# turtle-robotics/sea-current

Hardware: AMD Instinct MI355X
Metric: plans/sec (batched start-goal, 1024^2 grid) (higher is better)
Workload: dtype int32; 1 GPU; 1024x1024 random-obstacle grids (salt20, one grid and one query block per step), EDT + A*, 1024 batched queries per GPU and step, 10 steps = 10240 queries per library call; queries_per_launch=10240, map=salt20, queries_per_gpu=1024, queries_total=1024, lmax=4096, parallelism=query-sharded x1, contexts_in_flight=2, steps_per_call=10, hw_queues=4

## Files before the change

### include/sea_current_hip.h

```cpp
#ifndef SEA_CURRENT_HIP_H
#define SEA_CURRENT_HIP_H
#include <stdint.h>
#ifdef __cplusplus
extern "C" {
#endif

#define SC_ABI_VERSION 1

typedef struct sc_ctx sc_ctx;

typedef enum {
    SC_OK = 0,
    SC_ERR_INVALID = 1,
    SC_ERR_HIP = 2,
    SC_ERR_NOMEM = 3,
    SC_ERR_NO_DEVICE = 4
} sc_status;

typedef enum {
    SC_Q_OK = 0,
    SC_Q_NO_PATH = 1,
    SC_Q_BAD_ENDPOINT = 2,
    SC_Q_TRUNCATED = 3,
    SC_Q_RING_OVERFLOW = 4,
// ... 31 lines not shown
int sc_ctx_set_stream(sc_ctx* ctx, void* hip_stream);
int sc_ctx_use_own_stream(sc_ctx* ctx);
int sc_ctx_synchronize(sc_ctx* ctx);
int sc_ctx_set_timing(sc_ctx* ctx, int enable);
int sc_ctx_reset_timing(sc_ctx* ctx);
int sc_ctx_get_timing(sc_ctx* ctx, int kernel_id, double* total_ms, int64_t* launches);
int sc_ctx_scratch_bytes(sc_ctx* ctx, int64_t* bytes);

int sc_edt_u8_i32(sc_ctx* ctx, const uint8_t* occ, int W, int H, int batch, int32_t* d2);
int sc_edt_u8_i32_host(sc_ctx* ctx, const uint8_t* occ, int W, int H, int batch, int32_t* d2);

int sc_edt_nearest_i32(sc_ctx* ctx, const uint8_t* occ, const int32_t* d2, int W, int H, int batch, int32_t* nearest);

int sc_occ_from_rects(sc_ctx* ctx, const uint8_t* base, const int32_t* rects, int R, int W, int H, int free_border, uint8_t* occ);

int sc_occ_from_polygons(sc_ctx* ctx, const uint8_t* base, int G, int W, int H, float x_min, float y_min, float res_x, float res_y,
                         const float* lines, int n_lines, const int32_t* obs_off, int n_obs, const float* obs_box,
                         const uint8_t* obs_closed, const int32_t* grid_off, uint8_t* occ);
int sc_occ_from_polygons_host(sc_ctx* ctx, const uint8_t* base, int G, int W, int H, float x_min, float y_min, float res_x,
                              float res_y, const float* lines, int n_lines, const int32_t* obs_off, int n_obs, const float* obs_box,
                              const uint8_t* obs_closed, const int32_t* grid_off, uint8_t* occ);

int sc_moves_i32_u8(sc_ctx* ctx, const int32_t* d2, int W, int H, int32_t r2_clear, uint8_t* moves);

int sc_astar_batch(sc_ctx* ctx, const int32_t* d2, int W, int H, int32_t r2_clear,
                   const int32_t* start, const int32_t* goal, int Q, int Lmax,
                   int32_t* path, int32_t* len, int32_t* cost, int32_t* status);
int sc_astar_batch_host(sc_ctx* ctx, const int32_t* d2, int W, int H, int32_t r2_clear,
                        const int32_t* start, const int32_t* goal, int Q, int Lmax,
                        int32_t* path, int32_t* len, int32_t* cost, int32_t* status);
int sc_astar_batch_multi(sc_ctx* ctx, const int32_t* d2, int G, const int32_t* qgrid, int W, int H, int32_t r2_clear,
                         const int32_t* start, const int32_t* goal, int Q, int Lmax,
                         int32_t* path, int32_t* len, int32_t* cost, int32_t* status);
int sc_astar_last_expansions(sc_ctx* ctx, int64_t* expansions);
int sc_astar_debug_stats(sc_ctx* ctx, int32_t* stats4, int Q);
int sc_astar_debug_peek(sc_ctx* ctx, int32_t* out16);
int sc_astar_gfield(sc_ctx* ctx, const int32_t* d2, int W, int H, int32_t r2_clear,
                    int32_t start, int32_t goal, uint32_t* gfield, int32_t* cost, int32_t* status);

#define SC_FIELD_INF INT32_MAX
int sc_cost_field_batch(sc_ctx* ctx, const int32_t* d2, int G, const int32_t* fgrid, int W, int H, int32_t r2_clear,
                        const int32_t* root, int F, int rounds, int32_t* g, int32_t* fstatus);
int sc_cost_field_batch_host(sc_ctx* ctx, const int32_t* d2, int G, const int32_t* fgrid, int W, int H, int32_t r2_clear,
                             const int32_t* root, int F, int rounds, int32_t* g, int32_t* fstatus);
int sc_field_paths_batch(sc_ctx* ctx, const int32_t* d2, int G, const int32_t* fgrid, int W, int H, int32_t r2_clear,
                         const int32_t* g, const int32_t* root, int F, const int32_t* qfield, const int32_t* target, int Q,
// ... 406 lines not shown
```

### sea-current_amd/csrc/astar.hip

```cpp
#include "sc_internal.h"
#include <stdlib.h>

#define NBUCKET 32
#define ASTAR_CQ_THROUGHPUT 1024
#define ASTAR_RU_THROUGHPUT 4
#define ASTAR_CQ_LATENCY 2048
#define ASTAR_RU_LATENCY 8
#define E_RUN (1u << 18)
#define E_START (4u << 13 | 3u << 16)
#define RUNK 8

struct astar_args {
    const uint8_t* moves;
    const int32_t* d2;
    int W, H;
    int32_t rmin;
    const int32_t* start;
    const int32_t* goal;
    const int32_t* qgrid;
    const int32_t* order;
    const int32_t* nq_dev;
    int nq;
    int Lmax;
    int32_t* path;
    int32_t* len;
    int32_t* cost;
    int32_t* status;
    void* g;
    uint32_t* closed;
    uint32_t* buckets;
    int cap;
    int32_t* expanded;
    int32_t* counter;
    int32_t* ovf_list;
    int32_t* ovf_count;
    int32_t* ovf_sticky;
    int nstat;
    int lazy;
    int tw, bw;
    size_t gcells, bwords;
};

__device__ __forceinline__ int octile(int x, int y, int gx, int gy) {
    int dx = abs(x - gx), dy = abs(y - gy);
    return 10 * max(dx, dy) + 4 * min(dx, dy);
}

__device__ __forceinline__ uint32_t gix(int x, int y, int tw) {
    return ((((uint32_t)(y >> 2) * (uint32_t)tw + (uint32_t)(x >> 2)) << 4) | ((uint32_t)(y & 3) << 2)) | (uint32_t)(x & 3);
}
__device__ __forceinline__ uint32_t gix8(int x, int y, int tw8) {
    return ((((uint32_t)(y >> 3) * (uint32_t)tw8 + (uint32_t)(x >> 3)) << 6) | ((uint32_t)(y & 7) << 3)) | (uint32_t)(x & 7);
}
template <typename GT> __device__ __forceinline__ uint32_t gidx(int x, int y, int tw);
template <> __device__ __forceinline__ uint32_t gidx<uint32_t>(int x, int y, int tw) { return gix(x, y, tw); }
template <> __device__ __forceinline__ uint32_t gidx<uint8_t>(int x, int y, int tw) { return gix8(x, y, tw); }
__device__ __forceinline__ uint32_t cix(int x, int y, int bw) {
    return (((uint32_t)(y >> 4) * (uint32_t)bw + (uint32_t)(x >> 5)) << 4) | (uint32_t)(y & 15);
}

template <typename T>
__device__ __forceinline__ T g_load(const T* p) {
    return __hip_atomic_load(p, __ATOMIC_RELAXED, __HIP_MEMORY_SCOPE_AGENT);
// ... 60 lines not shown
                 "global_load_ubyte %[m], %[ma], off\n\t"
                 "s_mov_b64 %[sv], exec\n\t"
                 "v_cmp_ne_u32_e32 vcc, 0, %[b]\n\t"
                 "s_and_b64 exec, %[sv], vcc\n\t"
                 "global_atomic_or %[o], %[a], %[b], off sc0\n\t"
                 "s_mov_b64 exec, %[sv]"
                 : [sv] "=&s"(sv), [o] "+v"(old), [m] "=&v"(pmv), [r0] "=&v"(rm[0]), [r1] "=&v"(rm[1]), [r2] "=&v"(rm[2]), [r3] "=&v"(rm[3]),
                   [r4] "=&v"(rm[4]), [r5] "=&v"(rm[5]), [r6] "=&v"(rm[6])
                 : [a] "v"(bit_addr), [b] "v"(bits), [ma] "v"(mv_addr), [p0] "v"(ra[0]), [p1] "v"(ra[1]), [p2] "v"(ra[2]), [p3] "v"(ra[3]),
                   [p4] "v"(ra[4]), [p5] "v"(ra[5]), [p6] "v"(ra[6])
                 : "vcc", "scc", "memory");
}
__device__ __forceinline__ void pop_run_wait_loads(uint32_t (&rm)[RUNK - 1], uint32_t& pmv, uint32_t& old) {
    asm volatile("s_waitcnt vmcnt(1)" : "+v"(pmv), "+v"(old), "+v"(rm[0]), "+v"(rm[1]), "+v"(rm[2]), "+v"(rm[3]), "+v"(rm[4]), "+v"(rm[5]), "+v"(rm[6]) : : "memory");
}
__device__ __forceinline__ void pop_pair_wait_load(uint32_t& pmv, uint32_t& old) { asm volatile("s_waitcnt vmcnt(1)" : "+v"(pmv), "+v"(old) : : "memory"); }

__device__ __forceinline__ void pop_loads_issue(const uint8_t* mv_addr, const uint32_t* w_addr, uint32_t& byte, uint32_t& word) {
    asm volatile("global_load_ubyte %0, %2, off\n\t"
                 "global_load_dword %1, %3, off sc1"
                 : "=&v"(byte), "=&v"(word) : "v"(mv_addr), "v"(w_addr) : "memory");
}
__device__ __forceinline__ void pop_loads_wait(uint32_t& byte, uint32_t& word) { asm volatile("s_waitcnt vmcnt(0)" : "+v"(byte), "+v"(word) : : "memory"); }
__device__ __forceinline__ void masked_or_noret(uint32_t* addr, uint32_t bits) {
    unsigned long long sv;
    asm volatile("s_mov_b64 %[sv], exec\n\t"
                 "v_cmp_ne_u32_e32 vcc, 0, %[b]\n\t"
                 "s_and_b64 exec, %[sv], vcc\n\t"
                 "global_atomic_or %[a], %[b], off\n\t"
                 "s_mov_b64 exec, %[sv]"
                 : [sv] "=&s"(sv) : [a] "v"(addr), [b] "v"(bits) : "vcc", "scc", "memory");
}

__device__ __forceinline__ uint32_t bcast_group8(uint32_t v) {
    const uint32_t q = (uint32_t)__builtin_amdgcn_update_dpp(0, (int)v, 0x00 , 0xF, 0xF, false);
    const uint32_t r = (uint32_t)__builtin_amdgcn_update_dpp(0, (int)q, 0x114 , 0xF, 0xF, false);
    return q | r;
}

#define HQ 256
#define ASTAR_SPIN_LIMIT (1 << 20)
template <typename GT, bool DUAL, int CQ, int REFILL_UNROLL>
__device__ __forceinline__ void astar_query(const astar_args& a, const int q, const int slot) {
    constexpr int REFILL = CQ / 2;
    __shared__ uint32_t qe[CQ + 64];
    __shared__ int s_head[NBUCKET];
    __shared__ int s_tail[NBUCKET];
    __shared__ uint32_t nd_xy[64];
    __shared__ uint32_t nd_mv[64];
    __shared__ uint16_t succ[512];
    __shared__ uint8_t prune_tbl[64];
    __shared__ uint32_t dup_tbl[DUAL ? 1024 + 64 : 1];
    __shared__ uint2 hq_rec[DUAL ? HQ + 64 : 1];
    __shared__ int hq_tail, hq_head, hq_clean, hq_stop, hq_ovf, hq_fcur, hq_found, hq_flush;
    constexpr int SCOPE = DUAL ? __HIP_MEMORY_SCOPE_WORKGROUP : __HIP_MEMORY_SCOPE_WAVEFRONT;
    const int lane = threadIdx.x & 63;
    const int wv = DUAL ? __builtin_amdgcn_readfirstlane((int)(threadIdx.x >> 6)) : 0;
    const int W = a.W, H = a.H;
    const size_t cells = (size_t)W * H;
    const int s = a.start[q], t = a.goal[q];
    int32_t* path = a.path + (size_t)q * a.Lmax;

    int out_st = SC_Q_OK, out_len = 0, out_cost = -1, nexp = 0, npop = 0, kcyc = 0, nstep = 0;
    const size_t grid_off = a.qgrid ? (size_t)a.qgrid[q] * cells : 0;
    const uint8_t* const mvs = a.moves + grid_off;
    const bool bad = s < 0 || t < 0 || (size_t)s >= cells || (size_t)t >= cells || a.d2[grid_off + s] < a.rmin || a.d2[grid_off + t] < a.rmin;
    if (bad) out_st = SC_Q_BAD_ENDPOINT;
    else if (s == t) {
        if (lane == 0 && wv == 0) path[0] = s;
        out_len = 1; out_cost = 0; nexp = 1;
    } else {
    const int tw = a.tw, bw = a.bw;
    GT* g = static_cast<GT*>(a.g) + (size_t)slot * a.gcells;
    uint32_t* cl = a.closed + (size_t)slot * a.bwords;
    uint32_t* bk = a.buckets + (size_t)slot * NBUCKET * a.cap;
    const int cap = a.cap, capm = a.cap - 1;
    const int sx = s % W, sy = s / W, gx = t % W, gy = t / W;
    const int ddx[8] = {1, -1, 0, 0, 1, -1, 1, -1};
    const int ddy[8] = {0, 0, 1, -1, 1, 1, -1, -1};

    {
        uint4* p = reinterpret_cast<uint4*>(cl);
        const size_t n4 = a.bwords >> 2;
        for (size_t i = DUAL ? threadIdx.x : lane; i < n4; i += DUAL ? 128 : 64) p[i] = make_uint4(0, 0, 0, 0);
    }
    __builtin_amdgcn_wave_barrier();
    if (wv == 0 && lane < NBUCKET) { s_head[lane] = 0; s_tail[lane] = 0; }
    if (wv == 0) prune_tbl[lane] = (uint8_t)entry_prune((uint32_t)lane << 13);
// ... 217 lines not shown
                lt += n;
                if (lane == 0) __hip_atomic_store(&s_head[b], hd + n, __ATOMIC_RELAXED, SCOPE);
                wave_lds_sync();
            }
            const int n = min(64, lt - lh);
            npop += n; ++nstep;
            if (DUAL && n <= 16) {
                const int kl = n <= 4 ? 3 : n <= 8 ? 2 : n <= 16 ? 1 : 0, KL = 1 << kl, GL = 2 * KL;
                const int sub = lane >> (kl + 1), j = (lane >> kl) & 1, k = lane & (KL - 1);
                const bool valid = sub < n;
                const uint32_t e_raw = qe[(lh + sub) & (CQ - 1)];
                const uint32_t e = valid ? e_raw : 0u;
                lh += n;
                const int x = e & 0x1FFF, y = e >> 19;
                const uint32_t bit = 1u << (x & 31);
                const int dxg = gx - x, dyg = gy - y, adx = abs(dxg), ady = abs(dyg);
                const int dD = 4 + ((dxg < 0 ? 1 : 0) | (dyg < 0 ? 2 : 0));
                const int dS = adx > ady ? (dxg < 0 ? 1 : 0) : (dyg < 0 ? 3 : 2);
                const uint32_t bD = adx >= 1 && ady >= 1 ? 1u << dD : 0u, bS = adx != ady ? 1u << dS : 0u;
                const int d = j ? dS : dD;
                const bool has = valid && (j ? bS : bD) != 0u;
                const int lgeom = j ? abs(adx - ady) : min(adx, ady);
                const int ddx_ = (int)((0x2252u >> (2 * d)) & 3u) - 1, ddy_ = (int)((0x0A25u >> (2 * d)) & 3u) - 1;
                const uint8_t* const addr = mvs + (y * W + x) + (has ? min(k, lgeom - 1) : 0) * (ddy_ * W + ddx_);
                const bool head = valid && j == 0 && k == 0;
                uint32_t old, byte;
                uint32_t* const wa = &cl[cix(x, y, bw)];
                pop_loads_issue(addr, wa, byte, old);
                const uint32_t prune = prune_tbl[(e >> 13) & 63u];
                const int dup = dup_settle(head, x, y, e);
                pop_loads_wait(byte, old);
                const bool link = has && k < lgeom && ((byte >> d) & 1u) && (k > 0 || !((prune >> d) & 1u));
                const unsigned long long lm = __ballot(link);
                const uint32_t grp = (uint32_t)(lm >> (lane & ~(KL - 1))) & ((1u << KL) - 1u);
                const int run = __ffs((int)~grp) - 1;
                const uint32_t ne = entry_pack(x + (k + 1) * ddx_, y + (k + 1) * ddy_, d, byte) | (k + 1 < run ? E_RUN : 0u);
                const bool won1 = head && dup == 0 && !(old & bit);
                masked_or_noret(wa, won1 ? bit : 0u);
                const unsigned long long wm1 = __ballot(won1);
                const bool act = ((wm1 >> (lane & ~(GL - 1))) & 1ull) && k < run;
                {
                    const unsigned long long ma = __ballot(act);
                    if (ma) {
                        const int c = __popcll(ma);
                        if (__builtin_expect(lt - lh + c <= CQ, 1)) {
                            qe[act ? ((lt + (int)__builtin_amdgcn_mbcnt_hi((uint32_t)(ma >> 32), __builtin_amdgcn_mbcnt_lo((uint32_t)ma, 0u))) & (CQ - 1)) : CQ + lane] = ne;
                            lt += c;
                        } else push_entry(act, ne, 0);
                    }
                }
                hand_over(won1, x, y, (byte & ~prune) & ~(bD | bS), byte);
                nexp += __popcll(wm1);
            } else if (!DUAL && n <= 8) {
                const int sub = lane >> 3, d = lane & 7;
                const bool valid = sub < n;
                const uint32_t e = valid ? qe[(lh + sub) & (CQ - 1)] : 0u;
                lh += n;
                const int x = e & 0x1FFF, y = e >> 19;
                const uint32_t bit = 1u << (x & 31);
                uint32_t old = 0, pmv;
                const int hc = octile(x, y, gx, gy);
// ... 17 lines not shown
                    if (run == k && k < lmax && ((rm[k - 1] >> d) & 1u)) run = k + 1;
                const uint32_t ne = entry_pack(nx, ny, d, pmv) | (run > 1 ? E_RUN : 0u);
                atomic_wait(old);
                old = bcast_group8(old);
                const bool won = valid && !(old & bit);
                push_entry(won && cand, ne, df);
#pragma unroll
                for (int k = 2; k <= RUNK; ++k) {
                    if (__ballot(won && run >= k) == 0) break;
                    push_entry(won && run >= k, entry_pack(x + k * mdx, y + k * mdy, d, rm[k - 2]) | (run > k ? E_RUN : 0u), 0);
                }
                nexp += __popcll(__ballot(won && d == 0));
                if (__ballot(won && x == gx && y == gy)) found = true;
                if (won && d == 0) g[gidx<GT>(x, y, tw)] = (GT)(fcur - hc);
            } else if (DUAL) {
                const bool valid = lane < n;
                const uint32_t e_raw = qe[(lh + lane) & (CQ - 1)];
                const uint32_t e = valid ? e_raw : 0u;
                lh += n;
                const int x = e & 0x1FFF, y = e >> 19;
                const uint32_t bit = 1u << (x & 31);
                uint32_t old, pmv;
                uint32_t* const wa = &cl[cix(x, y, bw)];
                pop_loads_issue(mvs + (y * W + x), wa, pmv, old);
                const int dup = dup_settle(valid, x, y, e);
                const uint32_t prune = prune_tbl[(e >> 13) & 63u];
                const int dxg = gx - x, dyg = gy - y, adx = abs(dxg), ady = abs(dyg);
                const int dD = 4 + ((dxg < 0 ? 1 : 0) | (dyg < 0 ? 2 : 0));
                const int dS = adx > ady ? (dxg < 0 ? 1 : 0) : (dyg < 0 ? 3 : 2);
                const uint32_t bD = adx >= 1 && ady >= 1 ? 1u << dD : 0u, bS = adx != ady ? 1u << dS : 0u;
                const int nxD = x + (dxg < 0 ? -1 : 1), nyD = y + (dyg < 0 ? -1 : 1);
                const int nxS = x + (adx > ady ? (dxg < 0 ? -1 : 1) : 0), nyS = y + (adx > ady ? 0 : (dyg < 0 ? -1 : 1));
                pop_loads_wait(pmv, old);
                const uint32_t cand = valid ? (pmv & ~prune) : 0u;
                const uint32_t neD = (uint32_t)nyD << 19 | (uint32_t)dD << 13 | (uint32_t)nxD;
                const uint32_t neS = entry_pack(nxS, nyS, dS, pmv);
                const bool won = valid && dup == 0 && !(old & bit);
                masked_or_noret(wa, won ? bit : 0u);
                {
                    const bool pD = won && (cand & bD), pS = won && (cand & bS);
                    const unsigned long long mD = __ballot(pD), mS = __ballot(pS);
                    const int cD = __popcll(mD), c2 = cD + __popcll(mS);
                    if (c2) {
                        if (__builtin_expect(lt - lh + c2 <= CQ, 1)) {
                            qe[pD ? ((lt + (int)__builtin_amdgcn_mbcnt_hi((uint32_t)(mD >> 32), __builtin_amdgcn_mbcnt_lo((uint32_t)mD, 0u))) & (CQ - 1)) : CQ + lane] = neD;
                            qe[pS ? ((lt + cD + (int)__builtin_amdgcn_mbcnt_hi((uint32_t)(mS >> 32), __builtin_amdgcn_mbcnt_lo((uint32_t)mS, 0u))) & (CQ - 1)) : CQ + lane] = neS;
                            lt += c2;
                        } else {
                            push_entry(pD, neD, 0);
                            push_entry(pS, neS, 0);
                        }
                    }
                }
                nexp += __popcll(hand_over(won, x, y, cand & ~(bD | bS), pmv));
            } else {
                const bool valid = lane < n;
                const uint32_t e = valid ? qe[(lh + lane) & (CQ - 1)] : 0u;
                lh += n;
                const int x = e & 0x1FFF, y = e >> 19;
                const uint32_t bit = 1u << (x & 31);
                uint32_t old = 0, pmv;
// ... 147 lines not shown
            }
            out_len = L; out_cost = fcur;
        }
    }
    kcyc = (int)((__builtin_amdgcn_s_memtime() - t_begin) >> 10);
    }
    if (lane == 0 && wv == 0) {
        a.status[q] = out_st; a.len[q] = out_len; a.cost[q] = out_cost;
        a.expanded[q] = nexp; a.expanded[a.nstat + q] = npop; a.expanded[2 * a.nstat + q] = kcyc; a.expanded[3 * a.nstat + q] = nstep;
    }
}

template <typename GT>
__global__ void __launch_bounds__(64) astar_kernel(astar_args a) {
    const int nq = a.nq_dev ? *a.nq_dev : a.nq;
    for (;;) {
        const int qi = __builtin_amdgcn_readfirstlane(atomicAdd(a.counter, 1)) >> 6;
        if (qi >= nq) break;
        astar_query<GT, false, ASTAR_CQ_THROUGHPUT, ASTAR_RU_THROUGHPUT>(a, a.order ? a.order[qi] : qi, (int)blockIdx.x);
    }
}

template <typename GT, int CQ, int RU>
__global__ void __launch_bounds__(128) astar_kernel_dual(astar_args a) {
    __shared__ int s_qi;
    const int nq = a.nq_dev ? *a.nq_dev : a.nq;
    for (;;) {
        if (threadIdx.x == 0) s_qi = atomicAdd(a.counter, 64) >> 6;
        __syncthreads();
        const int qi = __builtin_amdgcn_readfirstlane(s_qi);
        __syncthreads();
        if (qi >= nq) break;
        astar_query<GT, true, CQ, RU>(a, a.order ? a.order[qi] : qi, (int)blockIdx.x);
        __syncthreads();
    }
}

__global__ void __launch_bounds__(1024) astar_prep_kernel(const int32_t* __restrict__ start, const int32_t* __restrict__ goal, int Q, int W,
                                                          int H, int32_t* __restrict__ order, int32_t* __restrict__ ctr) {
    __shared__ int hist[1024];
    __shared__ int scan[1024];
    const int tid = threadIdx.x;
    if (tid < 4) ctr[tid] = 0;
    if (!order) return;
    hist[tid] = 0;
    __syncthreads();
    const int hmax = 14 * max(W, H) + 1;
// ... 92 lines not shown
    if (slots * gcells * gsz > ctx->gslots.bytes || slots * bwords * 4 > ctx->closed.bytes || ring_slots(slots) * NBUCKET * (size_t)cap * 4 > ctx->buckets.bytes) {
        size_t free_b = 0, total_b = 0;
        if (hipMemGetInfo(&free_b, &total_b) == hipSuccess) {
            const size_t avail = (size_t)(0.9 * (double)(free_b + ctx->gslots.bytes + ctx->closed.bytes + ctx->buckets.bytes));
            while (slots > 1 && slots * (gcells * gsz + bwords * 4) + ring_slots(slots) * NBUCKET * (size_t)cap * 4 > avail) slots = (slots + 1) / 2;
        }
    }
    for (;;) {
        r = sc_scratch_reserve(ctx, &ctx->gslots, slots * gcells * gsz);
        if (r == SC_OK) r = sc_scratch_reserve(ctx, &ctx->closed, slots * bwords * 4);
        if (r == SC_OK) r = sc_scratch_reserve(ctx, &ctx->buckets, ring_slots(slots) * NBUCKET * (size_t)cap * 4);
        if (r == SC_OK) break;
        if (r != SC_ERR_NOMEM || slots <= 1) return r;
        (void)hipGetLastError();
        slots = (slots + 1) / 2;
    }
    if (!ctx->actr.p) {
        r = sc_scratch_reserve(ctx, &ctx->actr, 16 * sizeof(int32_t));
        if (r != SC_OK) return r;
        SC_HIP(ctx, hipMemsetAsync(ctx->actr.p, 0, 16 * sizeof(int32_t), ctx->stream));
    }
    int32_t* ctr = (int32_t*)ctx->actr.p;
    ctx->status_armed = true;

    const bool sorted = (size_t)Q > slots;
    int tk = sc_time_begin(ctx, SC_K_ASTAR);
    hipLaunchKernelGGL(astar_prep_kernel, dim3(1), dim3(1024), 0, ctx->stream, start, goal, Q, W, H, sorted ? order : (int32_t*)nullptr, ctr);
    astar_args a{(const uint8_t*)ctx->moves.p, d2, W, H, rmin, start, goal, qgrid, sorted ? order : nullptr, nullptr, Q, Lmax, path, len,
                 cost, status, ctx->gslots.p, (uint32_t*)ctx->closed.p, (uint32_t*)ctx->buckets.p, cap, expanded, ctr,
                 ovf_list, ctr + 1, ctx->status + SC_ST_ASTAR_OVERFLOW, Q, (dual && (size_t)Q > slots) ? 1 : 0, tw, bw, gcells, bwords};
    if (full_g) hipLaunchKernelGGL(astar_kernel<uint32_t>, dim3((unsigned)slots), dim3(64), 0, ctx->stream, a);
    else if (dual && latency && (size_t)Q <= slots)
        hipLaunchKernelGGL((astar_kernel_dual<uint8_t, ASTAR_CQ_LATENCY, ASTAR_RU_LATENCY>), dim3((unsigned)slots), dim3(128), 0, ctx->stream, a);
    else if (dual)
        hipLaunchKernelGGL((astar_kernel_dual<uint8_t, ASTAR_CQ_THROUGHPUT, ASTAR_RU_THROUGHPUT>), dim3((unsigned)slots), dim3(128), 0, ctx->stream, a);
    else hipLaunchKernelGGL(astar_kernel<uint8_t>, dim3((unsigned)slots), dim3(64), 0, ctx->stream, a);
    {
        const size_t rslots = slots >= 16 ? slots / 16 : 1;
        const int rcap = cap * 16;
        astar_args b = a;
        b.order = ovf_list; b.nq_dev = ctr + 1; b.nq = 0; b.cap = rcap; b.counter = ctr + 2;
        b.ovf_list = order; b.ovf_count = ctr + 3;
        if (full_g) hipLaunchKernelGGL(astar_kernel<uint32_t>, dim3((unsigned)rslots), dim3(64), 0, ctx->stream, b);
        else hipLaunchKernelGGL(astar_kernel<uint8_t>, dim3((unsigned)rslots), dim3(64), 0, ctx->stream, b);
    }
    sc_time_end(ctx, tk);
    SC_HIP(ctx, hipGetLastError());
    return SC_OK;
}

extern "C" int sc_astar_batch(sc_ctx* ctx, const int32_t* d2, int W, int H, int32_t r2_clear,
                              const int32_t* start, const int32_t* goal, int Q, int Lmax,
                              int32_t* path, int32_t* len, int32_t* cost, int32_t* status) {
// ... 69 lines not shown
```

### sea-current_amd/csrc/moves.hip

```cpp
#include "sc_internal.h"

__global__ void __launch_bounds__(256)
moves_kernel(const int32_t* __restrict__ d2, int W, int Hall, int H, int32_t rmin, uint8_t* __restrict__ moves) {
    const int x = blockIdx.x * 256 + threadIdx.x;
    const int yall = blockIdx.y;
    if (x >= W) return;
    const int y = yall % H;
    const int32_t* r1 = d2 + (size_t)yall * W;
    bool t[3][3];
#pragma unroll
    for (int j = -1; j <= 1; ++j)
#pragma unroll
        for (int i = -1; i <= 1; ++i) {
            int xx = x + i, yy = y + j;
            t[j + 1][i + 1] = xx >= 0 && xx < W && yy >= 0 && yy < H && r1[(ptrdiff_t)j * W + xx] >= rmin;
        }
    uint32_t m = 0;
    if (t[1][1]) {
        m |= (uint32_t)t[1][2] << 0;
        m |= (uint32_t)t[1][0] << 1;
        m |= (uint32_t)t[2][1] << 2;
        m |= (uint32_t)t[0][1] << 3;
        m |= (uint32_t)(t[2][2] && t[1][2] && t[2][1]) << 4;
        m |= (uint32_t)(t[2][0] && t[1][0] && t[2][1]) << 5;
// ... 73 lines not shown
    }
}

int sc_launch_moves(sc_ctx* ctx, const int32_t* d2, int W, int Hall, int H, int32_t r2, uint8_t* moves) {
    int32_t rmin = r2 > 1 ? r2 : 1;
    int tk = sc_time_begin(ctx, SC_K_MOVES);
    if (W % 4 == 0 && H % 4 == 0 && ((uintptr_t)d2 & 15) == 0 && ((uintptr_t)moves & 3) == 0)
        hipLaunchKernelGGL(moves4x4_kernel, dim3((W / 4 + 255) / 256, Hall / 4), dim3(256), 0, ctx->stream, d2, W, Hall, H, rmin, moves);
    else if (W % 4 == 0 && ((uintptr_t)d2 & 15) == 0 && ((uintptr_t)moves & 3) == 0)
        hipLaunchKernelGGL(moves4_kernel, dim3((W / 4 + 255) / 256, Hall), dim3(256), 0, ctx->stream, d2, W, Hall, H, rmin, moves);
    else
        hipLaunchKernelGGL(moves_kernel, dim3((W + 255) / 256, Hall), dim3(256), 0, ctx->stream, d2, W, Hall, H, rmin, moves);
    sc_time_end(ctx, tk);
    SC_HIP(ctx, hipGetLastError());
    return SC_OK;
}

extern "C" int sc_moves_i32_u8(sc_ctx* ctx, const int32_t* d2, int W, int H, int32_t r2_clear, uint8_t* moves) {
    if (!ctx || !d2 || !moves || W <= 0 || H <= 0 || W > SC_MAX_DIM || H > SC_MAX_DIM) return SC_ERR_INVALID;
    SC_HIP(ctx, hipSetDevice(ctx->device));
    return sc_launch_moves(ctx, d2, W, H, H, r2_clear, moves);
}

__host__ __device__ static inline int64_t isqrt64(int64_t v) {
    int64_t r = (int64_t)sqrt((double)v);
    while (r * r > v) --r;
    while ((r + 1) * (r + 1) <= v) ++r;
    return r;
}

__global__ void __launch_bounds__(256)
clearance_penalty_kernel(const int32_t* __restrict__ d2, size_t n, int32_t thr, int32_t r2_soft, int64_t s10, int pen_max,
                         uint8_t* __restrict__ pen) {
    const size_t i = (size_t)blockIdx.x * 256 + threadIdx.x;
    if (i >= n) return;
    const int32_t d = d2[i];
    uint8_t p = 0;
    if (d >= thr && d < r2_soft) p = (uint8_t)(((int64_t)pen_max * (s10 - isqrt64(100ll * d))) / s10);
    pen[i] = p;
}

extern "C" int sc_clearance_penalty_u8(sc_ctx* ctx, const int32_t* d2, int W, int H, int batch, int32_t r2_clear, int32_t r2_soft,
                                       int pen_max, uint8_t* pen) {
    if (!ctx || !d2 || !pen || W <= 0 || H <= 0 || W > SC_MAX_DIM || H > SC_MAX_DIM || batch <= 0 || pen_max < 0 || pen_max > 255 ||
        r2_soft < 1)
        return SC_ERR_INVALID;
// ... 25 lines not shown
```

### sea-current_amd/csrc/sc_internal.h

```cpp
#pragma once
#include <hip/hip_runtime.h>
#include <math.h>
#include <stdint.h>
#include <stdio.h>
#include <string.h>

#include <set>
#include <vector>

#include "../../include/sea_current_hip.h"

struct sc_scratch {
    void* p = nullptr;
    size_t bytes = 0;
    sc_scratch() = default;
    sc_scratch(const sc_scratch&) = delete;
    sc_scratch& operator=(const sc_scratch&) = delete;
    ~sc_scratch() { if (p) (void)hipFree(p); }
};

static inline size_t al256(size_t b) { return (b + 255) & ~(size_t)255; }

enum sc_status_word {
    SC_ST_ASTAR_OVERFLOW,
// ... 4 lines not shown
};

struct __attribute__((visibility("hidden"))) sc_ctx {
    int device = 0;
    hipStream_t own_stream = nullptr;
    hipStream_t stream = nullptr;
    hipEvent_t wait_ev = nullptr;
    int32_t *status = nullptr, *status_host = nullptr;
    bool status_armed = false;
    char err[256] = {0};
    int timing = 0;
    struct pending_ev { int kid; hipEvent_t a, b; bool shared_a = false; };
    std::vector<pending_ev> pending;
    std::vector<hipEvent_t> ev_pool;
    double t_ms[SC_K_COUNT] = {0};
    int64_t t_n[SC_K_COUNT] = {0};
    size_t scratch_total = 0;
    sc_scratch host_stage;
    sc_scratch astar_ends;
    sc_scratch colbits;
    sc_scratch updown;
    sc_scratch edt_flags;
    sc_scratch moves;
    sc_scratch gslots;
    sc_scratch closed;
    sc_scratch buckets;
    sc_scratch qstats;
    sc_scratch actr;
    sc_scratch bez_tang;
    sc_scratch bez_gl;
    sc_scratch bez_seginfo;
    sc_scratch cheb_a;
    sc_scratch fmt_nbr;
    sc_scratch gather_msg;
    sc_scratch wp_spill;
    sc_scratch sm_ctrl;
    sc_scratch sm_cum;
    sc_scratch sm_tp;
    sc_scratch sm_int;
    sc_scratch sm_smp;
    sc_scratch sm_vlim;
    sc_scratch occ_prep;
    sc_scratch fld_mask;
    sc_scratch fld_state;
    sc_scratch cmp_state;
    sc_scratch cmp_start;
// ... 70 lines not shown
    int upload();
    template <class T> T* dev(int i) const { return (T*)((char*)ctx_->host_stage.p + off_[i]); }
    int finish(int r);

  private:
    struct copy { int slot; void* host; size_t bytes; };
    int slot(size_t bytes) {
        off_.push_back(end_);
        end_ += al256(bytes ? bytes : 1);
        return (int)off_.size() - 1;
    }
    sc_ctx* ctx_;
    size_t end_ = 0;
    std::vector<size_t> off_;
    std::vector<copy> up_, down_;
};

int sc_time_begin(sc_ctx* ctx, int kid);
void sc_time_end(sc_ctx* ctx, int token);
int sc_time_chain(sc_ctx* ctx, int token, int kid);

int sc_launch_edt(sc_ctx* ctx, const uint8_t* occ, int W, int H, int batch, int32_t* d2);
int sc_launch_moves(sc_ctx* ctx, const int32_t* d2, int W, int Hall, int H, int32_t r2, uint8_t* moves);
int sc_launch_arclength(sc_ctx* ctx, const float* ctrl, int S, int nsub, float* cum, float* seg_len, const int32_t* S_dev);
int sc_launch_resample(sc_ctx* ctx, const float* ctrl, const float* cum, const float* arclength, const int32_t* seg_off, int B, int S,
                       int nsub, float* profile_pos, const int32_t* prof_off, int nudge, float* pts, float* tpar, int32_t* seg,
                       float* curvature, int32_t* status, const int32_t* S_dev);
struct sc_speed_frame {
    const int32_t* d2;
    int W, H;
    float x_min, y_min, res_x, res_y;
};
static inline bool sc_frame_ok(const sc_speed_frame& fr) {
    return fr.W >= 1 && fr.W <= SC_MAX_DIM && fr.H >= 1 && fr.H <= SC_MAX_DIM && isfinite(fr.x_min) && isfinite(fr.y_min) &&
           isfinite(fr.res_x) && fr.res_x > 0.f && isfinite(fr.res_y) && fr.res_y > 0.f;
}
int sc_launch_speed_limits(sc_ctx* ctx, const float* ctrl, const float* cum, const int32_t* seg_off, const float* arclength,
                           const int32_t* status, int P, int nsub, int N, int J, const double* limits, const double* dyn,
                           const sc_speed_frame& fr, int ns_bound, double* vlo, double* vhi, double* vhi_copy, float* min_clear,
                           int32_t* status_out);
int sc_speed_args_ok(int J, const double* dyn, const sc_speed_frame& fr);
int sc_speed_dyn_ok(const double* dyn, int P);
int sc_curve_grid_ok(const sc_speed_frame& fr, int32_t r2_clear);
int sc_launch_curve_clear(sc_ctx* ctx, const float* ctrl_in, float* ctrl_out, const int32_t* seg_off, const int32_t* status, int P,
                          const sc_speed_frame& fr, int32_t r2_clear, int max_level, uint8_t* level, int32_t* rounds, int32_t* leg_min,
                          int32_t* status_out);
// ... 31 lines not shown
```

### sea-current_amd/python/sea_current_amd/__init__.py

```python
import ctypes as C
import os
import re
import subprocess

import numpy as np

_PKG = os.path.dirname(os.path.abspath(__file__))
NATIVE_DIR = os.path.normpath(os.path.join(_PKG, "..", ".."))
REPO_ROOT = os.path.normpath(os.path.join(NATIVE_DIR, ".."))
LIB_PATH = os.environ.get("SC_LIB_PATH") or os.path.join(NATIVE_DIR, "libsea_current_hip.so")
HEADER_PATH = os.path.join(REPO_ROOT, "include", "sea_current_hip.h")

EDT_INF = 2**31 - 1
FIELD_INF = 2**31 - 1
FIELD_SEED_COST_MAX = 1 << 24
Q_OK, Q_NO_PATH, Q_BAD_ENDPOINT, Q_TRUNCATED, Q_RING_OVERFLOW, Q_BAD_PATH = 0, 1, 2, 3, 4, 5
K_EDT_COLBITS, K_EDT_BAND, K_MOVES, K_ASTAR, K_TOPPRA, K_TOPPRA_SAMPLE, K_BEZIER, K_ARCLENGTH, K_RESAMPLE, K_OCC, K_NEAREST, K_FMT, K_GATHER = range(13)
K_WAYPOINTS = 13
K_SMOOTH = 14
SMOOTH_OK, SMOOTH_BAD_INPUT, SMOOTH_NONFINITE, SMOOTH_TOPPRA_FAILED, SMOOTH_TRUNCATED, SMOOTH_EMPTY_SEGMENT = range(6)
SMOOTH_COLLIDES = 6
CURVE_MAX_LEGS, CURVE_MAX_LEVEL = 1024, 30
TRAJ_OK, TRAJ_SKIPPED, TRAJ_BAD = range(3)
TRAJ_MAX_TICKS = 65535
# ... 271 lines not shown
        import torch
        assert occ.is_cuda and occ.dtype == torch.uint8
        return self._edt(_on(occ.device), occ.contiguous(), out)

    def edt_host(self, occ):
        return self._edt(_HOST, occ)

    def _edt(self, A, occ, out=None):
        occ = A.arr(occ, A.u8)
        o3 = occ if len(occ.shape) == 3 else occ[None]
        B, H, W = o3.shape
        if out is None:
            out = A.new(tuple(o3.shape), A.i32)
        self._call("sc_edt_u8_i32" + A.suffix, _ptr(o3), W, H, B, _ptr(out))
        return out if len(occ.shape) == 3 else out.reshape(H, W)

    def moves(self, d2, r2=0):
        import torch
        H, W = d2.shape
        out = torch.empty((H, W), dtype=torch.uint8, device=d2.device)
        self._ck(self._l.sc_moves_i32_u8(self._h, _ptr(d2), W, H, r2, _ptr(out)), "sc_moves_i32_u8")
        return out

    def astar_batch(self, d2, start, goal, r2=0, Lmax=4096, out=None, label=None):
        return self._astar_batch(_on(d2.device), d2, start, goal, r2, Lmax, out, label)

    def astar_batch_host(self, d2, start, goal, r2=0, Lmax=4096):
        return self._astar_batch(_HOST, d2, start, goal, r2, Lmax)

    def _astar_batch(self, A, d2, start, goal, r2, Lmax, out=None, label=None):
        d2, start, goal = A.arr(d2, A.i32), A.arr(start, A.i32), A.arr(goal, A.i32)
        H, W = d2.shape
        Q = start.shape[0]
        if out is None:
            out = A.paths_out(Q, Lmax)
        res = [_ptr(out[k]) for k in ("path", "len", "cost", "status")]
        if label is not None:
            self._call("sc_astar_batch_screened", _ptr(d2), _ptr(label), 1, None, W, H, r2, _ptr(start), _ptr(goal), Q, Lmax, *res)
        else:
            self._call("sc_astar_batch" + A.suffix, _ptr(d2), W, H, r2, _ptr(start), _ptr(goal), Q, Lmax, *res)
        return out

    def astar_batch_multi(self, d2, qgrid, start, goal, r2=0, Lmax=4096, out=None, label=None):
        G, H, W = d2.shape
        Q = start.shape[0]
        if out is None:
# ... 1194 lines not shown
```

Baseline: 732,600 plans/s.

## Replace per-cell moves bytes with packed traversability bit tiles in throughput A*

Adds a kernel that packs the clearance test into 30x14 bit tiles with halo rows (16 words per tile). The throughput dual A* path then loads three adjacent row words with one dwordx3 load and rebuilds the 8-direction move mask in registers, instead of reading the precomputed moves byte. The goal is a denser, more cache-friendly neighbour lookup, paid for with an extra tile-building launch per call, extra ALU work per pop and extra scratch memory. It also sets waves_per_eu to 6 on the throughput kernel to raise occupancy.

Result: slower. 703,300 plans/s (-4.0%).

```diff
diff --git a/include/sea_current_hip.h b/include/sea_current_hip.h
--- a/include/sea_current_hip.h
+++ b/include/sea_current_hip.h
@@ -77,6 +77,8 @@
                               const uint8_t* obs_closed, const int32_t* grid_off, uint8_t* occ);
 
 int sc_moves_i32_u8(sc_ctx* ctx, const int32_t* d2, int W, int H, int32_t r2_clear, uint8_t* moves);
+
+int sc_trav_tiles_i32_u32(sc_ctx* ctx, const int32_t* d2, int W, int H, int G, int32_t r2_clear, uint32_t* tiles);
 
 int sc_astar_batch(sc_ctx* ctx, const int32_t* d2, int W, int H, int32_t r2_clear,
                    const int32_t* start, const int32_t* goal, int Q, int Lmax,
diff --git a/sea-current_amd/csrc/astar.hip b/sea-current_amd/csrc/astar.hip
--- a/sea-current_amd/csrc/astar.hip
+++ b/sea-current_amd/csrc/astar.hip
@@ -1,4 +1,5 @@
 #include "sc_internal.h"
+#include "trav_tiles.h"
 #include <stdlib.h>
 
 #define NBUCKET 32
@@ -39,6 +40,9 @@
     int lazy;
     int tw, bw;
     size_t gcells, bwords;
+    const uint32_t* trav;
+    int tpr;
+    uint32_t trav_words;
 };
 
 __device__ __forceinline__ int octile(int x, int y, int gx, int gy) {
@@ -145,6 +149,14 @@
                  : "=&v"(byte), "=&v"(word) : "v"(mv_addr), "v"(w_addr) : "memory");
 }
 __device__ __forceinline__ void pop_loads_wait(uint32_t& byte, uint32_t& word) { asm volatile("s_waitcnt vmcnt(0)" : "+v"(byte), "+v"(word) : : "memory"); }
+typedef uint32_t u32x3 __attribute__((ext_vector_type(3)));
+__device__ __forceinline__ int opaque(int v) { asm volatile("" : "+v"(v)); return v; }
+__device__ __forceinline__ void pop_loads_issue(const uint32_t* t_addr, const uint32_t* w_addr, u32x3& rows, uint32_t& word) {
+    asm volatile("global_load_dwordx3 %0, %2, off\n\t"
+                 "global_load_dword %1, %3, off sc1"
+                 : "=&v"(rows), "=&v"(word) : "v"(t_addr), "v"(w_addr) : "memory");
+}
+__device__ __forceinline__ void pop_loads_wait(u32x3& rows, uint32_t& word) { asm volatile("s_waitcnt vmcnt(0)" : "+v"(rows), "+v"(word) : : "memory"); }
 __device__ __forceinline__ void masked_or_noret(uint32_t* addr, uint32_t bits) {
     unsigned long long sv;
     asm volatile("s_mov_b64 %[sv], exec\n\t"
@@ -187,6 +199,9 @@
     int out_st = SC_Q_OK, out_len = 0, out_cost = -1, nexp = 0, npop = 0, kcyc = 0, nstep = 0;
     const size_t grid_off = a.qgrid ? (size_t)a.qgrid[q] * cells : 0;
     const uint8_t* const mvs = a.moves + grid_off;
+    constexpr bool TRAV = DUAL && CQ == ASTAR_CQ_THROUGHPUT;
+    const uint32_t* const trv = TRAV ? a.trav + (a.qgrid ? (size_t)a.qgrid[q] * a.trav_words : 0) : nullptr;
+    const uint32_t tpr = TRAV ? (uint32_t)a.tpr : 0u;
     const bool bad = s < 0 || t < 0 || (size_t)s >= cells || (size_t)t >= cells || a.d2[grid_off + s] < a.rmin || a.d2[grid_off + t] < a.rmin;
     if (bad) out_st = SC_Q_BAD_ENDPOINT;
     else if (s == t) {
@@ -450,21 +465,27 @@
                 const bool has = valid && (j ? bS : bD) != 0u;
                 const int lgeom = j ? abs(adx - ady) : min(adx, ady);
                 const int ddx_ = (int)((0x2252u >> (2 * d)) & 3u) - 1, ddy_ = (int)((0x0A25u >> (2 * d)) & 3u) - 1;
-                const uint8_t* const addr = mvs + (y * W + x) + (has ? min(k, lgeom - 1) : 0) * (ddy_ * W + ddx_);
+                const uint8_t* const addr = TRAV ? nullptr : mvs + (y * W + x) + (has ? min(k, lgeom - 1) : 0) * (ddy_ * W + ddx_);
                 const bool head = valid && j == 0 && k == 0;
                 uint32_t old, byte;
                 uint32_t* const wa = &cl[cix(x, y, bw)];
-                pop_loads_issue(addr, wa, byte, old);
+                u32x3 rows;
+                const int kk = has ? min(k, lgeom - 1) : 0;
+                if constexpr (TRAV) pop_loads_issue(trv + tt_cell((uint32_t)(x + kk * ddx_), (uint32_t)(y + kk * ddy_), tpr), wa, rows, old);
+                else pop_loads_issue(addr, wa, byte, old);
                 const uint32_t prune = prune_tbl[(e >> 13) & 63u];
                 const int dup = dup_settle(head, x, y, e);
-                pop_loads_wait(byte, old);
+                if constexpr (TRAV) {
+                    pop_loads_wait(rows, old);
+                    byte = tt_moves_from_pack((uint32_t)opaque((int)tt_pack(rows.x, rows.y, rows.z, tt_shift((uint32_t)(opaque(x) + kk * ddx_)))));
+                } else pop_loads_wait(byte, old);
                 const bool link = has && k < lgeom && ((byte >> d) & 1u) && (k > 0 || !((prune >> d) & 1u));
                 const unsigned long long lm = __ballot(link);
                 const uint32_t grp = (uint32_t)(lm >> (lane & ~(KL - 1))) & ((1u << KL) - 1u);
                 const int run = __ffs((int)~grp) - 1;
                 const uint32_t ne = entry_pack(x + (k + 1) * ddx_, y + (k + 1) * ddy_, d, byte) | (k + 1 < run ? E_RUN : 0u);
                 const bool won1 = head && dup == 0 && !(old & bit);
-                masked_or_noret(wa, won1 ? bit : 0u);
+                masked_or_noret(TRAV ? &cl[cix(opaque(x), y, bw)] : wa, won1 ? bit : 0u);
                 const unsigned long long wm1 = __ballot(won1);
                 const bool act = ((wm1 >> (lane & ~(GL - 1))) & 1ull) && k < run;
                 {
@@ -528,7 +549,9 @@
                 const uint32_t bit = 1u << (x & 31);
                 uint32_t old, pmv;
                 uint32_t* const wa = &cl[cix(x, y, bw)];
-                pop_loads_issue(mvs + (y * W + x), wa, pmv, old);
+                u32x3 rows;
+                if constexpr (TRAV) pop_loads_issue(trv + tt_cell((uint32_t)x, (uint32_t)y, tpr), wa, rows, old);
+                else pop_loads_issue(mvs + (y * W + x), wa, pmv, old);
                 const int dup = dup_settle(valid, x, y, e);
                 const uint32_t prune = prune_tbl[(e >> 13) & 63u];
                 const int dxg = gx - x, dyg = gy - y, adx = abs(dxg), ady = abs(dyg);
@@ -537,12 +560,15 @@
                 const uint32_t bD = adx >= 1 && ady >= 1 ? 1u << dD : 0u, bS = adx != ady ? 1u << dS : 0u;
                 const int nxD = x + (dxg < 0 ? -1 : 1), nyD = y + (dyg < 0 ? -1 : 1);
                 const int nxS = x + (adx > ady ? (dxg < 0 ? -1 : 1) : 0), nyS = y + (adx > ady ? 0 : (dyg < 0 ? -1 : 1));
-                pop_loads_wait(pmv, old);
+                if constexpr (TRAV) {
+                    pop_loads_wait(rows, old);
+                    pmv = tt_moves_from_pack((uint32_t)opaque((int)tt_pack(rows.x, rows.y, rows.z, tt_shift((uint32_t)opaque(x)))));
+                } else pop_loads_wait(pmv, old);
                 const uint32_t cand = valid ? (pmv & ~prune) : 0u;
                 const uint32_t neD = (uint32_t)nyD << 19 | (uint32_t)dD << 13 | (uint32_t)nxD;
                 const uint32_t neS = entry_pack(nxS, nyS, dS, pmv);
                 const bool won = valid && dup == 0 && !(old & bit);
-                masked_or_noret(wa, won ? bit : 0u);
+                masked_or_noret(TRAV ? &cl[cix(opaque(x), y, bw)] : wa, won ? bit : 0u);
                 {
                     const bool pD = won && (cand & bD), pS = won && (cand & bS);
                     const unsigned long long mD = __ballot(pD), mS = __ballot(pS);
@@ -736,7 +762,8 @@
 }
 
 template <typename GT, int CQ, int RU>
-__global__ void __launch_bounds__(128) astar_kernel_dual(astar_args a) {
+__global__ void __launch_bounds__(128) __attribute__((amdgpu_waves_per_eu(CQ == ASTAR_CQ_THROUGHPUT ? 6 : 1)))
+astar_kernel_dual(astar_args a) {
     __shared__ int s_qi;
     const int nq = a.nq_dev ? *a.nq_dev : a.nq;
     for (;;) {
@@ -875,13 +902,23 @@
     }
     int32_t* ctr = (int32_t*)ctx->actr.p;
     ctx->status_armed = true;
+    const bool throughput = dual && !(latency && (size_t)Q <= slots);
+    const size_t trav_words = tt_words(W, H);
+    if (throughput) {
+        if (trav_words > 0xFFFFFFFFull) return SC_ERR_INVALID;
+        r = sc_scratch_reserve(ctx, &ctx->trav, trav_words * (size_t)G * 4);
+        if (r != SC_OK) return r;
+        r = sc_launch_trav_tiles(ctx, d2, W, H, G, r2, (uint32_t*)ctx->trav.p);
+        if (r != SC_OK) return r;
+    }
 
     const bool sorted = (size_t)Q > slots;
     int tk = sc_time_begin(ctx, SC_K_ASTAR);
     hipLaunchKernelGGL(astar_prep_kernel, dim3(1), dim3(1024), 0, ctx->stream, start, goal, Q, W, H, sorted ? order : (int32_t*)nullptr, ctr);
     astar_args a{(const uint8_t*)ctx->moves.p, d2, W, H, rmin, start, goal, qgrid, sorted ? order : nullptr, nullptr, Q, Lmax, path, len,
                  cost, status, ctx->gslots.p, (uint32_t*)ctx->closed.p, (uint32_t*)ctx->buckets.p, cap, expanded, ctr,
-                 ovf_list, ctr + 1, ctx->status + SC_ST_ASTAR_OVERFLOW, Q, (dual && (size_t)Q > slots) ? 1 : 0, tw, bw, gcells, bwords};
+                 ovf_list, ctr + 1, ctx->status + SC_ST_ASTAR_OVERFLOW, Q, (dual && (size_t)Q > slots) ? 1 : 0, tw, bw, gcells, bwords,
+                 throughput ? (const uint32_t*)ctx->trav.p : nullptr, tt_tiles_x(W), (uint32_t)trav_words};
     if (full_g) hipLaunchKernelGGL(astar_kernel<uint32_t>, dim3((unsigned)slots), dim3(64), 0, ctx->stream, a);
     else if (dual && latency && (size_t)Q <= slots)
         hipLaunchKernelGGL((astar_kernel_dual<uint8_t, ASTAR_CQ_LATENCY, ASTAR_RU_LATENCY>), dim3((unsigned)slots), dim3(128), 0, ctx->stream, a);
diff --git a/sea-current_amd/csrc/moves.hip b/sea-current_amd/csrc/moves.hip
--- a/sea-current_amd/csrc/moves.hip
+++ b/sea-current_amd/csrc/moves.hip
@@ -1,4 +1,5 @@
 #include "sc_internal.h"
+#include "trav_tiles.h"
 
 __global__ void __launch_bounds__(256)
 moves_kernel(const int32_t* __restrict__ d2, int W, int Hall, int H, int32_t rmin, uint8_t* __restrict__ moves) {
@@ -119,6 +120,67 @@
     return sc_launch_moves(ctx, d2, W, H, H, r2_clear, moves);
 }
 
+template <bool VEC>
+__global__ void __launch_bounds__(256)
+trav_tiles_kernel(const int32_t* __restrict__ d2, int W, int H, int G, int32_t rmin, int tpr, int tyn, uint32_t* __restrict__ tiles) {
+    const int nbx = (tpr + 63) >> 6, vrows = TT_H * tyn + 2;
+    const int tx = (int)(blockIdx.x % (unsigned)nbx) * 64 + (int)(threadIdx.x & 63);
+    const long long rowall = (long long)(blockIdx.x / (unsigned)nbx) * 4 + (threadIdx.x >> 6);
+    if (tx >= tpr || rowall >= (long long)G * vrows) return;
+    const int gi = (int)(rowall / vrows), v = (int)(rowall % vrows) - 1;
+    uint32_t word = 0;
+    if (v >= 0 && v < H) {
+        const int32_t* r = d2 + ((size_t)gi * H + v) * W;
+        const int c0 = TT_W * tx - 1;
+        if (VEC) {
+            const int a0 = c0 & ~3;
+            unsigned long long bits = 0;
+#pragma unroll
+            for (int k = 0; k < 9; ++k) {
+                const int c = a0 + 4 * k;
+                if (c >= 0 && c < W) {
+                    const int4 q = *reinterpret_cast<const int4*>(r + c);
+                    const uint32_t nib = (uint32_t)(q.x >= rmin) | (uint32_t)(q.y >= rmin) << 1 | (uint32_t)(q.z >= rmin) << 2 | (uint32_t)(q.w >= rmin) << 3;
+                    bits |= (unsigned long long)nib << (4 * k);
+                }
+            }
+            word = (uint32_t)(bits >> (c0 - a0));
+        } else {
+            for (int b = 0; b < 32; ++b) {
+                const int c = c0 + b;
+                if (c >= 0 && c < W && r[c] >= rmin) word |= 1u << b;
+            }
+        }
+    }
+    uint32_t* const t0 = tiles + (size_t)gi * tpr * tyn * 16;
+    const int ty = (v + TT_H) / TT_H - 1, rr = v - TT_H * ty;
+    if (ty >= 0 && ty < tyn) t0[((size_t)ty * tpr + tx) * 16 + rr + 1] = word;
+    if (rr == TT_H - 1 && ty + 1 < tyn) t0[((size_t)(ty + 1) * tpr + tx) * 16] = word;
+    if (rr == 0 && ty >= 1) t0[((size_t)(ty - 1) * tpr + tx) * 16 + 15] = word;
+}
+
+int sc_launch_trav_tiles(sc_ctx* ctx, const int32_t* d2, int W, int H, int G, int32_t r2, uint32_t* tiles) {
+    const int32_t rmin = r2 > 1 ? r2 : 1;
+    const int tpr = tt_tiles_x(W), tyn = tt_tiles_y(H);
+    const long long rows = (long long)G * (TT_H * tyn + 2), blocks = (long long)((tpr + 63) >> 6) * ((rows + 3) / 4);
+    if (blocks > 0x7FFFFFFFll) return SC_ERR_INVALID;
+    int tk = sc_time_begin(ctx, SC_K_MOVES);
+    if (W % 4 == 0 && ((uintptr_t)d2 & 15) == 0)
+        hipLaunchKernelGGL(trav_tiles_kernel<true>, dim3((unsigned)blocks), dim3(256), 0, ctx->stream, d2, W, H, G, rmin, tpr, tyn, tiles);
+    else
+        hipLaunchKernelGGL(trav_tiles_kernel<false>, dim3((unsigned)blocks), dim3(256), 0, ctx->stream, d2, W, H, G, rmin, tpr, tyn, tiles);
+    sc_time_end(ctx, tk);
+    SC_HIP(ctx, hipGetLastError());
+    return SC_OK;
+}
+
+extern "C" int sc_trav_tiles_i32_u32(sc_ctx* ctx, const int32_t* d2, int W, int H, int G, int32_t r2_clear, uint32_t* tiles) {
+    if (!ctx || !d2 || !tiles || W <= 0 || H <= 0 || G <= 0 || W > SC_MAX_DIM || H > SC_MAX_DIM || (long long)H * G > 0x7FFFFFFF / W)
+        return SC_ERR_INVALID;
+    SC_HIP(ctx, hipSetDevice(ctx->device));
+    return sc_launch_trav_tiles(ctx, d2, W, H, G, r2_clear, tiles);
+}
+
 __host__ __device__ static inline int64_t isqrt64(int64_t v) {
     int64_t r = (int64_t)sqrt((double)v);
     while (r * r > v) --r;
diff --git a/sea-current_amd/csrc/sc_internal.h b/sea-current_amd/csrc/sc_internal.h
--- a/sea-current_amd/csrc/sc_internal.h
+++ b/sea-current_amd/csrc/sc_internal.h
@@ -50,6 +50,7 @@
     sc_scratch updown;
     sc_scratch edt_flags;
     sc_scratch moves;
+    sc_scratch trav;
     sc_scratch gslots;
     sc_scratch closed;
     sc_scratch buckets;
@@ -166,6 +167,7 @@
 
 int sc_launch_edt(sc_ctx* ctx, const uint8_t* occ, int W, int H, int batch, int32_t* d2);
 int sc_launch_moves(sc_ctx* ctx, const int32_t* d2, int W, int Hall, int H, int32_t r2, uint8_t* moves);
+int sc_launch_trav_tiles(sc_ctx* ctx, const int32_t* d2, int W, int H, int G, int32_t r2, uint32_t* tiles);
 int sc_launch_arclength(sc_ctx* ctx, const float* ctrl, int S, int nsub, float* cum, float* seg_len, const int32_t* S_dev);
 int sc_launch_resample(sc_ctx* ctx, const float* ctrl, const float* cum, const float* arclength, const int32_t* seg_off, int B, int S,
                        int nsub, float* profile_pos, const int32_t* prof_off, int nudge, float* pts, float* tpar, int32_t* seg,
diff --git a/sea-current_amd/csrc/trav_tiles.h b/sea-current_amd/csrc/trav_tiles.h
--- /dev/null
+++ b/sea-current_amd/csrc/trav_tiles.h
@@ -0,0 +1,37 @@
+#pragma once
+#include <stddef.h>
+#include <stdint.h>
+
+#if defined(__HIPCC__) || defined(__CUDACC__)
+#define TT_HD __host__ __device__ __forceinline__
+#else
+#define TT_HD static inline
+#endif
+
+#define TT_W 30
+#define TT_H 14
+#define TT_MAX_COORD 8200
+
+TT_HD uint32_t tt_div30(uint32_t x) { return (x * 8739u) >> 18; }
+TT_HD uint32_t tt_div14(uint32_t y) { return (y * 9363u) >> 17; }
+TT_HD int tt_tiles_x(int W) { return (W + TT_W - 1) / TT_W; }
+TT_HD int tt_tiles_y(int H) { return (H + TT_H - 1) / TT_H; }
+TT_HD size_t tt_words(int W, int H) { return (size_t)tt_tiles_x(W) * (size_t)tt_tiles_y(H) * 16; }
+
+TT_HD uint32_t tt_shift(uint32_t x) { return x - TT_W * tt_div30(x); }
+TT_HD uint32_t tt_cell(uint32_t x, uint32_t y, uint32_t tpr) {
+    const uint32_t tx = tt_div30(x), ty = tt_div14(y);
+    return ((ty * tpr + tx) << 4) + (y - TT_H * ty);
+}
+
+TT_HD uint32_t tt_moves_byte(uint32_t a, uint32_t c, uint32_t b) {
+    const uint32_t E = (c >> 2) & 1u, Wt = c & 1u, S = (b >> 1) & 1u, N = (a >> 1) & 1u;
+    const uint32_t m = E | Wt << 1 | S << 2 | N << 3 | (((b >> 2) & 1u) & E & S) << 4 | ((b & 1u) & Wt & S) << 5 | (((a >> 2) & 1u) & E & N) << 6 |
+                       ((a & 1u) & Wt & N) << 7;
+    return (c & 2u) ? m : 0u;
+}
+TT_HD uint32_t tt_pack(uint32_t w0, uint32_t w1, uint32_t w2, uint32_t shift) {
+    return ((w0 >> shift) & 7u) | ((w1 >> shift) & 7u) << 3 | ((w2 >> shift) & 7u) << 6;
+}
+TT_HD uint32_t tt_moves_from_pack(uint32_t n) { return tt_moves_byte(n, n >> 3, n >> 6); }
+TT_HD uint32_t tt_moves_from_words(uint32_t w0, uint32_t w1, uint32_t w2, uint32_t shift) { return tt_moves_from_pack(tt_pack(w0, w1, w2, shift)); }
diff --git a/sea-current_amd/python/sea_current_amd/__init__.py b/sea-current_amd/python/sea_current_amd/__init__.py
--- a/sea-current_amd/python/sea_current_amd/__init__.py
+++ b/sea-current_amd/python/sea_current_amd/__init__.py
@@ -317,6 +317,14 @@
         self._ck(self._l.sc_moves_i32_u8(self._h, _ptr(d2), W, H, r2, _ptr(out)), "sc_moves_i32_u8")
         return out
 
+    def trav_tiles(self, d2, r2=0):
+        import torch
+        d3 = d2 if d2.dim() == 3 else d2[None]
+        G, H, W = d3.shape
+        out = torch.empty((G, (H + 13) // 14, (W + 29) // 30, 16), dtype=torch.int32, device=d2.device)
+        self._ck(self._l.sc_trav_tiles_i32_u32(self._h, _ptr(d3), W, H, G, r2, _ptr(out)), "sc_trav_tiles_i32_u32")
+        return out
+
     def astar_batch(self, d2, start, goal, r2=0, Lmax=4096, out=None, label=None):
         return self._astar_batch(_on(d2.device), d2, start, goal, r2, Lmax, out, label)
 
```
